# tensor4all/tensor4all-rs

Hardware: AMD Instinct MI355X
Metric: TCI2 full-sweep GF/s (d=30, chi=256 fp64) (higher is better)
Workload: dtype f64

## Files before the change

tensor4all-rs_amd/csrc/engine.hip:

```cpp
#include "engine.hpp"

#include <algorithm>
#include <cmath>
#include <cstdio>
#include <cstdlib>
#include <cstring>
#include <atomic>
#include <condition_variable>
#include <mutex>

namespace t4a {

namespace {
thread_local std::string g_last_error;

__global__ void __launch_bounds__(256) tri_extract_kernel(const double* __restrict__ in, int ldi, int rows, int cols,
                                                          int keep_lower, int unit_diag, double* __restrict__ out,
                                                          int ldo)
{
    const int i = blockIdx.x * blockDim.x + threadIdx.x;
    if (i >= rows) return;
    for (int j = blockIdx.y; j < cols; j += gridDim.y) {
        double v;
        if (i == j)
// ... 249 lines not shown
    if (e != hipSuccess || count <= 0)
        throw Error(T4A_GPU_NO_DEVICE,
                    "no HIP device available: the tensor4all-rs MI355X backend has no CPU fallback (hipGetDeviceCount: " +
                        std::string(hipGetErrorString(e)) + ")");
}

void tri_extract_launch(const double* in, int ldi, int rows, int cols, int keep_lower, int unit_diag, double* out,
                        int ldo, hipStream_t stream)
{
    if (rows <= 0 || cols <= 0) return;
    dim3 grid((rows + 255) / 256, cols < 1024 ? cols : 1024);
    hipLaunchKernelGGL(tri_extract_kernel, grid, dim3(256), 0, stream, in, ldi, rows, cols, keep_lower, unit_diag, out,
                       ldo);
}

Engine::Engine()
{
    require_device();
    num_cus_ = pool::compute_units();
    stream_ = pool::stream_get(1);
    ev_rrlu_.init();
    ev_fac_.init();
    static const int xcc_env = std::getenv("T4A_XCD_ID") ? std::atoi(std::getenv("T4A_XCD_ID")) : -1;
    xcc_ = xcc_env >= 0 ? (xcc_env > 8 ? (xcc_env & 7) : xcc_env) : xcd_assign();
    g_live_engines.fetch_add(1, std::memory_order_relaxed);
    std::call_once(g_census_once, xcd_census);
}

Engine::~Engine()
{
    g_live_engines.fetch_sub(1, std::memory_order_relaxed);
    if (stream_) pool::stream_put(stream_, 1);
}

namespace {
int chain_max_steps(const RrluRoute& rt, size_t max_bond_dim)
{
    const int mn = rt.kM < rt.kN ? rt.kM : rt.kN;
    return max_bond_dim < (size_t)mn ? (int)max_bond_dim : mn;
}
void print_stamps(const RrluRoute& rt, int M, int N, int steps, const unsigned long long* hs)
{
    const double st = steps > 0 ? (double)steps : 1.0;
    switch (rt.kind) {
    case RrluKind::OneWave:
        std::fprintf(stderr, "[rrlu stamps w1] M=%d N=%d columns=%d steps=%d cycles/step: search=%.0f stop+divide+clear=%.0f tables=%.0f update=%.0f | launch (cycles): "
                             "load+init=%llu steps=%llu write-out=%llu | shader clock %.0f MHz\n",
                     M, N, rt.xcd.CPT, steps, hs[0] / st, hs[1] / st, hs[2] / st, hs[3] / st, hs[16], hs[17], hs[18], hs[21] ? 100.0 * (double)hs[20] / (double)hs[21] : 0.0);
        break;
    case RrluKind::OneWorkgroup:
    case RrluKind::SingleXcd:
    case RrluKind::MultiXcd:
        std::fprintf(stderr, "[rrlu stamps xcd] M=%d N=%d W=%d steps=%d cycles/step: pass=%.0f search=%.0f publish=%.0f | prefetch=%.0f keys=%.0f pick=%.0f slow+stop=%.0f recwr=%.0f barB=%.0f | record=%.0f "
                             "tables+u=%.0f colwait=%.0f divide=%.0f barC=%.0f lread=%.0f | pollspins=%llu exact sweeps=%llu exact picks=%llu | launch (cycles): election=%llu load+init=%llu steps=%llu write-out=%llu\n",
                     M, N, rt.xcd.W, steps, hs[0] / st, hs[1] / st, hs[2] / st, hs[6] / st, hs[8] / st, hs[14] / st, hs[15] / st, hs[9] / st, hs[3] / st, hs[10] / st, hs[11] / st, hs[12] / st,
                     hs[4] / st, hs[13] / st, hs[7] / st, hs[5], hs[22], hs[23], hs[16], hs[17], hs[18], hs[19]);
        break;
    default: {
        const bool reg = rt.kind == RrluKind::Reg;
        const int W = reg ? rt.reg.W : rt.kind == RrluKind::Lds ? rt.lds.W : rrlu_global_blocks(M, N);
        const int T = reg ? rt.reg.T : rt.kind == RrluKind::Lds ? rt.lds.T : 256;
        std::fprintf(stderr, "[rrlu stamps %s] M=%d N=%d W=%d T=%d steps=%d | s0=%llu s1=%llu s2=%llu s3=%llu s4=%llu pollspins=%llu colspins=%llu s7=%llu "
                             "(cycles, wg0/thread0; lds: publish,poll,colfetch,pass,reduce; reg: pass,reduce,publish,poll,fetch)\n",
                     reg ? "reg" : "lds", M, N, W, T, steps, hs[0], hs[1], hs[2], hs[3], hs[4], hs[5], hs[6], hs[7]);
    }
    }
}
}

RrluRoute Engine::luci_route(int M, int N, bool left) const
{
    const RrluEnv& env = rrlu_env();
    const bool huge = M > 65535 || N > 65535;
    const int kM = left ? M : N, kN = left ? N : M;
    if (!huge && !env.force_lds && !env.force_global && !env.force_reg && !nonfinite_retry_) {
        RrluXcdPlan xplan;
        if ((long)kM * kN > env.wg_min && (rrlu_w1_make_plan(kM, kN, &xplan, 0) || rrlu_wg_make_plan(kM, kN, &xplan, 0)))
            return RrluRoute::of_xcd(xplan, kM, kN);
        if (!xcd_disabled() && (rrlu_xcd_make_plan(kM, kN, &xplan, false, xcd_plan_max_w()) || rrlu_xcd_make_plan(kM, kN, &xplan, false, 32, true)))
            return RrluRoute::of_xcd(xplan, kM, kN);
    }
    RrluRegPlan rplan;
    if (!huge && !env.force_lds && !env.force_global && rrlu_reg_make_plan(kM, kN, num_cus_, &rplan)) return RrluRoute::of_reg(rplan, kM, kN);
    RrluRoute rt;
    rt.kM = M;
    rt.kN = N;
    if (!huge && !env.force_global) rt.lds = rrlu_make_plan(M, N, num_cus_);
    rt.kind = huge || env.force_global || rt.lds.lds_bytes > 160 * 1024 ? RrluKind::Global : RrluKind::Lds;
    return rt;
}

LuciResult Engine::luci(const double* d_a, int M, int N, const RrLUOptions& opts, bool need_factors, bool want_lu_copy,
                        const FusedPi* fused)
{
    const double* const d_a_in = d_a;
    LuciResult r;
    r.M = M;
    r.N = N;
    r.row_perm.resize(M);
    r.col_perm.resize(N);
    for (int i = 0; i < M; ++i) r.row_perm[i] = i;
    for (int j = 0; j < N; ++j) r.col_perm[j] = j;
    if (M == 0 || N == 0) {
        r.rank = 0;
        r.last_error = 0.0;
        r.pivot_errors = {0.0};
        r.has_factors = need_factors;
        return r;
    }
// ... 300 lines not shown
        const double rr = r.rank;
        prof.v[10] += (M - rr) * rr * rr + 2.0 * rr * rr * N;
        r.has_factors = true;
    }
    return r;
}

void Engine::xcd_take_tickets(const RrluXcdPlan& plan, RrluXcdArgs& a)
{
    if (plan.K > 1) {
        a.ticket = d_xticket_.get() + 8;
        a.ticket_base = xcd_ticket_base_multi_;
        xcd_ticket_base_multi_ += (unsigned)(plan.grid / 8);
    } else {
        a.ticket = d_xticket_.get();
        a.ticket_base = xcd_ticket_base_;
        if (!plan.wg) xcd_ticket_base_ += (unsigned)(plan.grid / 8);
    }
}

void Engine::xcd_mailbox_clear(size_t words, hipStream_t stream)
{
    d_xkeys_.reserve(words);
    d_xticket_.reserve(16);
    T4A_HIP(hipMemsetAsync(d_xkeys_.get(), 0, d_xkeys_.cap * sizeof(unsigned long long), stream));
    T4A_HIP(hipMemsetAsync(d_xticket_.get(), 0, 16 * sizeof(unsigned), stream));
    xcd_ticket_base_ = xcd_ticket_base_multi_ = 0;
    xcd_salt_ = 0;
}

void Engine::xcd_args(RrluXcdArgs& a, const RrluRoute& rt, bool left, const double* A, int max_steps, double rel_tol, double abs_tol,
                      const RrluBlock& blk, int xcc)
{
    std::memset(&a, 0, sizeof(a));
    a.A = A;
    a.M = rt.kM;
    a.N = rt.kN;
    a.max_steps = max_steps;
    a.rel_tol = rel_tol;
    a.abs_tol = abs_tol;
    a.tie_row_major = left ? 0 : 1;
    a.out_transposed = left ? 0 : 1;
    a.W = rt.xcd.W;
    a.xcc = xcc;
    xcd_take_tickets(rt.xcd, a);
    a.row_perm = left ? blk.row_perm() : blk.col_perm();
    a.col_perm = left ? blk.col_perm() : blk.row_perm();
    a.iresult = blk.iresult();
    a.dresult = blk.dresult();
    a.pivot_vals = blk.pivot_vals();
    a.keys = d_xkeys_.get();
    a.salt = xcd_salt_;
    a.spec_frac = 0.8;
    a.h_block = reinterpret_cast<unsigned long long*>(blk.host);
    a.block_u64 = (int)(blk.bytes / 8);
    a.ts_u64 = (int)(blk.off_ts / 8);
}

void Engine::rrlu_account(const RrluRoute& rt, bool tie_row_major, int M, int N, int rank, bool record, float ms, bool saturated)
{
    double bytes = 8.0 * M * N, flops = 0.0;
    for (int k = 0; k < rank; ++k) {
        const double mr = (double)(M - k - 1), nr = (double)(N - k - 1);
        bytes += 16.0 * mr * nr;
        flops += 2.0 * mr * nr + mr;
    }
    prof.v[8] += rank;
    prof.v[9] += bytes;
    prof.v[10] += flops;
    if (!record) return;
    auto add = [&](int code) {
        auto& vs = variant_stats_[code];
        vs[0] += ms;
        vs[1] += 1.0;
        vs[2] += bytes;
        vs[3] += rank;
    };
    add(rt.code(tie_row_major));
    if (saturated) add(rt.code(tie_row_major, true));
}

RrluRoute Engine::chain_route(int kM, int kN) const
{
    if (kM < 1 || kN < 1 || kM > 65535 || kN > 65535) return RrluRoute();
    RrluXcdPlan xplan;
    if ((long long)kM * kN > rrlu_env().wg_min && (rrlu_w1_make_plan(kM, kN, &xplan, 63) || rrlu_wg_make_plan(kM, kN, &xplan, 63)))
        return RrluRoute::of_xcd(xplan, kM, kN);
    RrluRegPlan rplan;
    if ((long long)kM * kN <= 64 * 64 && rrlu_reg_make_plan(kM, kN, num_cus_, &rplan) && rplan.W == 1) return RrluRoute::of_reg(rplan, kM, kN);
    if (!xcd_disabled() && (rrlu_xcd_make_plan(kM, kN, &xplan, true, xcd_plan_max_w()) || rrlu_xcd_make_plan(kM, kN, &xplan, true, 32, true)))
        return RrluRoute::of_xcd(xplan, kM, kN);
    return RrluRoute();
}

void Engine::chain_begin(const std::vector<RrluRoute>& routes, size_t reserve_mailbox_words)
{
    chain_group_reserve(routes, reserve_mailbox_words, stream_);
    RrluLock scope = RrluLock::None;
    for (const RrluRoute& rt : routes)
        if (rt.on_xcd()) scope = std::max(scope, rt.lock());
    acquire_for(chain_lock_, scope, xcc_);
}

void Engine::chain_end() { chain_lock_.release(); }

RrluRoute Engine::chain_group_route(int kM, int kN)
// ... 345 lines not shown
```

tensor4all-rs_amd/csrc/kernels.hpp:

```cpp
#pragma once

#include <hip/hip_runtime.h>

#include <cstddef>
#include <cstdint>

#include "../../include/t4a_testfunctions.h"

namespace t4a {

struct RrluWorkspace;

struct RrluPlan {
    int W = 1;
    int T = 256;
    int cpw = 0;
    int Mld = 0;
    size_t lds_bytes = 0;
};

RrluPlan rrlu_make_plan(int M, int N, int num_cus);

struct RrluArgs {
    const double* A;
// ... 95 lines not shown
    unsigned done_token;
    const int* dims;
    int dims_swap;
    unsigned dev_token;
    const int* rowmap;
    int ts_u64;
};
bool rrlu_reg_make_plan(int M, int N, int num_cus, RrluRegPlan* out);
size_t rrlu_reg_keys_bytes(const RrluRegPlan& plan);
size_t rrlu_reg_cols_bytes(const RrluRegPlan& plan, int M);
void rrlu_reg_launch(const RrluRegPlan& plan, const RrluRegArgs& args, hipStream_t stream, bool keys_zeroed = false);

struct XcdSpecArgs {
    double* out;
    const uint64_t* dep_acc;
    const uint64_t* w_site;
    const uint64_t* ext_acc;
    const int* ext_cnt;
    const uint64_t* ind_acc;
    const int* ind_cnt;
    unsigned* tile_counter;
    int total, d;
    FnDevice fn;
};
struct RrluXcdPlan {
    int W = 1;
    int RPT = 1, CPT = 1;
    int grid = 8;
    size_t lds_bytes = 0;
    int wg = 0;
    int K = 1;
    bool big() const { return K > 1 || RPT > 16; }
};
struct RrluXcdArgs {
    const double* A;
    double* Aout;
    double* urows;
    int M, N;
    int max_steps;
    double rel_tol, abs_tol;
    int tie_row_major;
    int out_transposed;
    int W;
    int xcc;
    unsigned* ticket;
    unsigned ticket_base;
    int* row_perm;
    int* col_perm;
    int* iresult;
    double* dresult;
    double* pivot_vals;
    unsigned long long* keys;
    unsigned salt;
    double spec_frac;
    unsigned long long* stamps;
    unsigned long long* h_block;
    int block_u64;
    const int* dims;
    int dims_swap;
    const int* rowmap;
    XcdSpecArgs spec;
    int ts_u64;
};
bool rrlu_xcd_make_plan(int M, int N, RrluXcdPlan* out, bool any_size = false, int max_w = 32, bool allow_big = false);
size_t rrlu_xcd_keys_bytes(const RrluXcdPlan& plan);
size_t rrlu_xcd_cols_bytes(const RrluXcdPlan& plan, int M);
struct RrluXcdGroupArgs {
    RrluXcdArgs p[8];
};
void rrlu_xcd2_launch(const RrluXcdPlan& plan, const RrluXcdArgs& args, hipStream_t stream);
void rrlu_xcd2m_launch(const RrluXcdPlan& plan, const RrluXcdArgs& args, hipStream_t stream);
void rrlu_xcd2_group_launch(const RrluXcdPlan& plan, const RrluXcdGroupArgs& args, bool tie_row_major, hipStream_t stream);
bool rrlu_wg_make_plan(int M, int N, RrluXcdPlan* out, int spec_blocks = 0);
void rrlu_wg_launch(const RrluXcdPlan& plan, const RrluXcdArgs& args, hipStream_t stream);
void rrlu_wg_group_launch(const RrluXcdPlan& plan, const RrluXcdGroupArgs& args, bool tie_row_major, hipStream_t stream);
bool rrlu_w1_make_plan(int M, int N, RrluXcdPlan* out, int spec_blocks = 0);
void rrlu_w1_launch(const RrluXcdPlan& plan, const RrluXcdArgs& args, hipStream_t stream);
void rrlu_w1_group_launch(const RrluXcdPlan& plan, const RrluXcdGroupArgs& args, bool tie_row_major, hipStream_t stream);

void pi_eval_launch(const FnDevice& fn, const uint64_t* rowacc, int M, const uint64_t* colacc, int N, double* out,
                    int ld, bool transpose_out, unsigned long long* max_abs_bits, hipStream_t stream);
struct PiJob {
    const uint64_t* rowacc;
    const uint64_t* colacc;
    double* out;
    unsigned long long* max_abs_bits;
    int M, N, ld, pad_;
};
void pi_eval_batched_launch(const FnDevice& fn, const PiJob* d_jobs, int n_jobs, int max_M, int max_N, hipStream_t stream);
struct PackJob {
    const double* src;
    double* core;
    const int* info;
    int ld, L, S, R, last, pad_;
};
struct LuProblem;
constexpr int FILL_SMALL_MAX_N = 32, FILL_SMALL_MAX_RHS = 64;
void fill_small_launch(const FnDevice& fn, const PiJob* d_pis, const LuProblem* d_lups, const PackJob* d_packs, int n_jobs, int last_site,
                       hipStream_t stream);
void stage_copy_launch(const uint64_t* pinned_src, uint64_t* dst, size_t count, hipStream_t stream);
void absmax_launch(const double* data, size_t count, unsigned long long* max_abs_bits, hipStream_t stream);

constexpr int CHAIN_MAX_SET = 1024;
struct ChainTab {
    uint64_t* code;
    uint64_t* acc;
// ... 290 lines not shown
```

tensor4all-rs_amd/csrc/kernels_rrlu_xcd2.hip:

```cpp
#include "kernels_rrlu_xcd_common.hpp"

namespace t4a {

namespace {

template <int RPT, int KX = 1> struct Xcd2Lds {
    static constexpr int LSTR = xcd_lstr(RPT);
    static constexpr int TBL = xcd2_tbl(RPT, KX);
    static constexpr int o_l = 0;
    static constexpr int o_wd = o_l + 64 * LSTR * 8;
    static constexpr int o_wi = o_wd + 16;
    static constexpr int o_pp = o_wi + 64;
    static constexpr int o_st = o_pp + 16;
    static constexpr int o_pv = o_st + 128;
    static constexpr int o_pr = o_pv + TBL * 8;
    static constexpr int o_rp = o_pr + TBL * 2;
    static constexpr int o_pc = o_rp + TBL * 2;
    static constexpr int o_cp = o_pc + TBL * 2;
    static constexpr int bytes = o_cp + TBL * 2;
};
static_assert(Xcd2Lds<12>::bytes == (int)xcd_lds_total(12), "plan.lds_bytes must cover the layout");
static_assert(Xcd2Lds<24>::bytes == (int)xcd2_lds_total(24), "plan.lds_bytes must cover the layout (plans beyond 1024 rows)");
static_assert(Xcd2Lds<16, 3>::bytes == (int)xcd2_lds_total(16, 3), "plan.lds_bytes must cover the layout (plans beyond 1024 columns)");

#ifndef T4A_XCD_STAMP_WAVE
#define T4A_XCD_STAMP_WAVE 0
#endif

constexpr unsigned X2_META_VALID = 1u << 13;
constexpr unsigned X2_ROW_MASK = 2047u;
constexpr int X2_QSHIFT = 11, X2_PSHIFT = 11;

constexpr int X2_DIVW = XWAVES - 1;

template <int R0, int NR, int RPT> __device__ __forceinline__ unsigned x2_colmax_hi(unsigned acc, const XSlab<RPT>& col)
{
#pragma unroll
    for (int r = 0; r + 1 < NR; r += 2) acc = vmax3_hi_abs(acc, hi32(col.get(R0 + r)), hi32(col.get(R0 + r + 1)));
    if constexpr ((NR & 1) != 0) acc = vmax3_hi_abs(acc, hi32(col.get(R0 + NR - 1)), hi32(col.get(R0 + NR - 1)));
    return acc;
}

template <int RPT, int CPT, bool ROWMAJOR, int KX = 1>
__device__ __forceinline__ void rrlu_xcd2_body(const RrluXcdArgs& p, const RrluXcdArgs* pk)
{
    static_assert(XWAVES == 8, "the second-generation kernel is written for eight waves per workgroup");
    static_assert(KX >= 1 && KX <= 3, "instantiated for up to three XCDs");
    constexpr int ST_AUX = KX > 1 ? BUF_SC1 : 0;
    extern __shared__ __attribute__((aligned(16))) char smem_raw[];
    using L = Xcd2Lds<RPT, KX>;
    constexpr int LSTR = L::LSTR;
    constexpr int MP = 64 * RPT;
    double* const lbuf = reinterpret_cast<double*>(smem_raw + L::o_l);
    int* const ctl = reinterpret_cast<int*>(smem_raw + L::o_wi);
    unsigned long long* const lds_ptrs = reinterpret_cast<unsigned long long*>(smem_raw + L::o_pp);
    unsigned long long* const lds_stamps = reinterpret_cast<unsigned long long*>(smem_raw + L::o_st);
    double* const lds_pivots = reinterpret_cast<double*>(smem_raw + L::o_pv);
    unsigned short* const posrow = reinterpret_cast<unsigned short*>(smem_raw + L::o_pr);
    unsigned short* const rowpos = reinterpret_cast<unsigned short*>(smem_raw + L::o_rp);
    unsigned short* const poscol = reinterpret_cast<unsigned short*>(smem_raw + L::o_pc);
    unsigned short* const colpos = reinterpret_cast<unsigned short*>(smem_raw + L::o_cp);

    const int tid = threadIdx.x;
    const int lane = tid & 63;
    const int wave = __builtin_amdgcn_readfirstlane(tid >> 6);
    const unsigned long long t_entry = (kXcdStamps && p.stamps) ? __builtin_amdgcn_s_memtime() : 0ull;

    if (tid == 0) {
        int rank = -1;
        if constexpr (KX == 1) {
            if ((int)xcc_id() == p.xcc) {
                const unsigned t = atomicAdd(p.ticket, 1u) - p.ticket_base;
                if (t < (unsigned)p.W) rank = (int)t;
            }
        } else {
            const unsigned x = xcc_id() & 7u;
            const unsigned t = atomicAdd(p.ticket + x, 1u) - p.ticket_base;
            const unsigned xi = (x - (unsigned)p.xcc) & 7u;
            if (xi < (unsigned)KX && t < (unsigned)p.W) rank = (int)(xi * (unsigned)p.W + t);
        }
        ctl[3] = rank;
        ctl[0] = 0;
        ctl[1] = 0;
        ctl[2] = 0;
        for (int e = 8; e < 16; ++e) ctl[e] = 0;
        lds_ptrs[0] = (unsigned long long)p.iresult;
        lds_ptrs[1] = (unsigned long long)p.h_block;
        for (int e = 0; e < 16; ++e) lds_stamps[e] = 0ull;
    }
    __syncthreads();
    const int rank = __builtin_amdgcn_readfirstlane(ctl[3]);
    if (rank < 0) {
        if (p.spec.out && p.dims) {
            const int m_spec = p.dims[2] != 0 ? 0 : (p.dims_swap ? p.dims[1] : p.dims[0]);
            if (m_spec > 0 && m_spec <= p.M)
                xcd_spec_work(reinterpret_cast<const XcdSpecArgs*>(kernarg_base() + offsetof(RrluXcdArgs, spec)), m_spec, ctl + 8);
        }
        return;
    }
    const unsigned long long ts_begin = p.ts_u64 > 0 ? wall_clock64() : 0ull;
    const unsigned long long t_elected = (kXcdStamps && p.stamps) ? __builtin_amdgcn_s_memtime() : 0ull;
    const int NWL = p.W * XWAVES;
    const int NW = KX * NWL;
    const int g = rank * XWAVES + wave;
    const bool poller = wave == 0;
    const int xi = KX > 1 ? rank / p.W : 0;
    const int pbase = xi * NWL;
    int M = p.M, N = p.N, max_steps = p.max_steps;
    int lda = p.M;
    if (p.dims) {
        const int d0 = __builtin_amdgcn_readfirstlane(p.dims[0]), d1 = __builtin_amdgcn_readfirstlane(p.dims[1]);
        M = p.dims_swap ? d1 : d0;
        N = p.dims_swap ? d0 : d1;
        if (M > p.M || N > p.N) M = N = 0;
        const int mn = M < N ? M : N;
        max_steps = max_steps < mn ? max_steps : mn;
        if (mn <= 0) return;
        lda = p.rowmap ? __builtin_amdgcn_readfirstlane(p.dims[3]) : M;
    }
    M = __builtin_amdgcn_readfirstlane(M);
    N = __builtin_amdgcn_readfirstlane(N);
    max_steps = __builtin_amdgcn_readfirstlane(max_steps);
    lda = __builtin_amdgcn_readfirstlane(lda);

    unsigned active = 0u;
#pragma unroll
    for (int q = 0; q < CPT; ++q)
        if (g + NW * q < N) active |= 1u << q;
    XSlab<RPT> a[CPT];
    double local_sqmax = 0.0;
    bool bad = false;
    int srow[RPT];
    unsigned rowmask = 0u;
#pragma unroll
    for (int r = 0; r < RPT; ++r) {
        const int i = lane + 64 * r;
        const bool rok = i < M;
// ... 12 lines not shown
#pragma unroll
    for (int q = 0; q < CPT; ++q) {
        const bool cok = g + NW * q < N;
        const unsigned rm = (unsigned)opaque_v((int)rowmask);
#pragma unroll
        for (int r = 0; r < RPT; ++r) {
            const bool ok = cok && ((rm >> r) & 1u);
            const double v = ok ? a[q].get(r) : 0.0;
            const double sqv = v * v;
            if (sqv > local_sqmax) local_sqmax = sqv;
            bad |= !((v - v) == 0.0);
            a[q].set(r, v);
        }
    }
    bad |= !(local_sqmax < __builtin_huge_val());
    for (int i = tid; i < M; i += XT) {
        posrow[i] = (unsigned short)i;
        rowpos[i] = (unsigned short)i;
    }
    for (int j = tid; j < N; j += XT) {
        poscol[j] = (unsigned short)j;
        colpos[j] = (unsigned short)j;
    }
    for (int e = tid; e < 64 * LSTR; e += XT) lbuf[e] = 0.0;
    {
        const double wm = wave_max_f64(sqrt(local_sqmax));
        if (lane == 0 && wm > 0.0)
            atomicMax((unsigned long long*)&p.dresult[1], (unsigned long long)__double_as_longlong(wm));
    }
    const unsigned wave_bad = __ballot(bad) != 0ull ? 1u : 0u;
    __syncthreads();

    const bool stamp_on = kXcdStamps && (p.stamps != nullptr) && rank == 0 && tid == 64 * T4A_XCD_STAMP_WAVE;
    unsigned long long stamp_last = stamp_on ? __builtin_amdgcn_s_memtime() : 0ull;
    const unsigned long long t_loop = stamp_last;

    const unsigned k2_base = 2u * (unsigned)NW * 16u;
    const unsigned cols_base = 4u * (unsigned)NW * 16u;
    const unsigned fin_base = cols_base + 2u * (unsigned)NW * (unsigned)(MP / 16) * 256u;
    const unsigned k3_base = fin_base + 256u;
    const __amdgpu_buffer_rsrc_t mail =
        __builtin_amdgcn_make_buffer_rsrc((void*)p.keys, 0, (int)(k3_base + (KX > 1 ? 2u * (unsigned)NW * 16u : 0u)), 0x00020000);

    int npiv = 0;
    double max_error = 0.0;
    double error = __builtin_nan("");
    bool timed_out = false;
    const double min_pivot_abs = (p.rel_tol == 0.0 && p.abs_tol == 0.0) ? 0.0 : 2.220446049250313e-16;
    double u[CPT];
#pragma unroll
    for (int q = 0; q < CPT; ++q) u[q] = 0.0;
    double prev_sq = __builtin_huge_val();
    double spec_frac = p.spec_frac, rel_tol_v = p.rel_tol, abs_tol_v = p.abs_tol;
    asm volatile("" : "+v"(spec_frac), "+v"(rel_tol_v), "+v"(abs_tol_v));
    constexpr unsigned XSPIN = 1u << 20;

    unsigned mq[CPT];
#pragma unroll
    for (int q = 0; q < CPT; ++q) mq[q] = (active & (1u << q)) ? x2_colmax_hi<0, RPT>(0u, a[q]) : 0u;
    [[maybe_unused]] unsigned long long n_exact_sweep = 0ull, n_exact_pick = 0ull;
    constexpr int XR = (RPT + X2_DIVW - 1) / X2_DIVW;
    const int sr0 = wave - 1;

    for (int kn = 0; kn < max_steps; ++kn) {
        const int k = kn - 1;
        const int par = kn & 1;
        const unsigned tag = (p.salt << 16) | (unsigned)(kn + 1);
        int mh = (int)mq[0];
#pragma unroll
        for (int q = 1; q < CPT; ++q) mh = (int)mq[q] > mh ? (int)mq[q] : mh;
        const int whi = wave_max_i32(mh);
        const int kslot = (par * NW + g) * 16;
        {
            u32x4 kv;
            kv.x = 0u;
            kv.y = (unsigned)whi;
            kv.z = wave_bad;
            kv.w = tag ^ kv.y ^ kv.z;
            if (lane == 0) __builtin_amdgcn_raw_buffer_store_b128(kv, mail, kslot, 0, 0);
        }
        u32x4 kg[4], kh[4];
        bool has_cand = false;
        double cval = 0.0;
        int cirow = 0, qstar = 0;
        double sq = 0.0;
        if (active != 0u) {
            bool done = false;
            if (hi_mid(whi)) {
                unsigned long long bq[CPT];
                int nhit = 0;
#pragma unroll
                for (int q = 0; q < CPT; ++q) {
                    bq[q] = __ballot(mq[q] == (unsigned)whi);
                    nhit += __builtin_popcountll(bq[q]);
                }
                if (nhit == 1) {
#pragma unroll
                    for (int q = 0; q < CPT; ++q)
                        if (bq[q] != 0ull) {
                            const int hl = (int)__builtin_ctzll(bq[q]);
                            unsigned bits = 0u;
#pragma unroll
                            for (int r = 0; r < RPT; ++r)
                                asm("v_cmp_eq_f32 vcc, |%1|, %2\n\tv_addc_co_u32 %0, vcc, %0, %0, vcc" : "+v"(bits) : "v"(hi32(a[q].get(r))), "s"(whi) : "vcc");
                            const unsigned hb_ = (unsigned)__builtin_amdgcn_readlane((int)bits, hl);
                            if (__builtin_popcount(hb_) == 1) {
                                const int rstar = RPT - 1 - (int)__builtin_ctz(hb_);
// ... 27 lines not shown
                    if (active & (1u << q)) {
                        const unsigned cp_ = colpos[opaque_s(g + NW * q)];
                        auto sweep = [&](int r, double av) {
                            const int i = lane_o + 64 * r;
                            const unsigned rp_ = rowpos[i < M_o ? i : 0];
                            const unsigned key = ROWMAJOR ? ((rp_ << X2_PSHIFT) | cp_) : ((cp_ << X2_PSHIFT) | rp_);
                            const double sc = av * av;
                            const bool hit = (i < M_o) & ((int)rp_ > k) & (sc == sq);
                            if (hit && key < mypos) {
                                mypos = key;
                                myval = av;
                                myrow = i;
                                myq = q;
                            }
                        };
                        if constexpr (RPT <= 16) {
#pragma unroll
                            for (int r = 0; r < RPT; ++r) sweep(r, a[q].get(r));
                        } else {
#pragma unroll 1
                            for (int r = 0; r < RPT; ++r) sweep(r, a[q].dyn(opaque_s(r)));
                        }
                    }
                }
                const unsigned wp = (unsigned)__builtin_amdgcn_readfirstlane((int)wave_min_u32(mypos));
                if (wp != XNOPOS) {
                    const unsigned long long sel = __ballot(mypos == wp);
                    const int hl = (int)__builtin_ctzll(sel);
                    has_cand = true;
                    cval = readlane_f64(myval, hl);
                    cirow = __builtin_amdgcn_readlane(myrow, hl);
                    qstar = __builtin_amdgcn_readlane(myq, hl);
                }
            }
        }
        XSTAMP(1);
        {
            const unsigned meta = (unsigned)cirow | ((unsigned)qstar << X2_QSHIFT) | (has_cand ? X2_META_VALID : 0u);
            u32x4 kv;
            kv.x = lo32(cval);
            kv.y = hi32(cval);
            kv.z = meta;
            kv.w = tag ^ kv.x ^ kv.y ^ meta;
            if (lane == 0) {
                __builtin_amdgcn_raw_buffer_store_b128(kv, mail, (int)k2_base + kslot, 0, 0);
                if constexpr (KX > 1) __builtin_amdgcn_raw_buffer_store_b128(kv, mail, (int)k3_base + kslot, 0, ST_AUX);
            }
        }
        if (poller) {
#pragma unroll
            for (int j = 0; j < 4; ++j)
                kg[j] = __builtin_amdgcn_raw_buffer_load_b128(mail, (par * NW + pbase + min(lane + 64 * j, NWL - 1)) * 16, 0, BUF_SC1);
        }
        const bool early_pub = !poller && has_cand && (sq >= spec_frac * prev_sq);
        constexpr int CS = 256, SLOTB = (MP / 16) * CS;
        const int myslot = (int)cols_base + (par * NW + g) * SLOTB + (lane >> 4) * CS + (lane & 15) * 16;
        if (early_pub) {
            if (qstar == 0) xcd_publish_column<0, RPT, ST_AUX>(a[0], mail, myslot, tag, 4 * CS);
            if constexpr (CPT > 1) if (qstar == 1) xcd_publish_column<1, RPT, ST_AUX>(a[1], mail, myslot, tag, 4 * CS);
            if constexpr (CPT > 2) if (qstar == 2) xcd_publish_column<2, RPT, ST_AUX>(a[2], mail, myslot, tag, 4 * CS);
            if constexpr (CPT > 3) if (qstar == 3) xcd_publish_column<3, RPT, ST_AUX>(a[3], mail, myslot, tag, 4 * CS);
        }
        XSTAMP(2);

        if (poller) {
            unsigned spins = 0;
            int giveup = 0;
            XSTAMP(6);
            for (;;) {
                bool ok = true;
#pragma unroll
                for (int j = 0; j < 4; ++j) ok &= ((kg[j].x ^ kg[j].y ^ kg[j].z ^ kg[j].w) == tag);
                if (__all(ok)) break;
                xcd_poll_again();
                if (++spins > XSPIN) {
                    giveup = 1;
                    break;
                }
#pragma unroll
                for (int j = 0; j < 4; ++j)
                    kg[j] = __builtin_amdgcn_raw_buffer_load_b128(mail, (par * NW + pbase + min(lane + 64 * j, NWL - 1)) * 16, 0, BUF_SC1);
            }
            if (stamp_on) lds_stamps[5] += spins;
            u32x4 fr;
            int xr = 0, fslot = 0;
            if constexpr (KX > 1) {
                fslot = (int)fin_base + (par * KX) * 16;
                xr = (lane < KX && lane != xi) ? lane : (xi == 0 ? 1 : 0);
                fr = __builtin_amdgcn_raw_buffer_load_b128(mail, fslot + xr * 16, 0, BUF_SC1);
            }
#pragma unroll
            for (int j = 0; j < 4; ++j)
                kh[j] = __builtin_amdgcn_raw_buffer_load_b128(mail, (int)k2_base + (par * NW + pbase + min(lane + 64 * j, NWL - 1)) * 16, 0, BUF_SC1);
            XSTAMP(8);
            int wa_ = 0;
            unsigned wkx = 0u, wky = 0u, wkz = 0u;
            if (!giveup) {
                if (kn == 0) {
                    unsigned zf = 0u;
#pragma unroll
                    for (int j = 0; j < 4; ++j) zf |= kg[j].z;
                    if (__ballot(zf != 0u) != 0ull) giveup = 2;
                }
                bool decided = false;
                int lh = (int)kg[0].y;
#pragma unroll
                for (int j = 1; j < 4; ++j) lh = (int)kg[j].y > lh ? (int)kg[j].y : lh;
                const int ghi = wave_max_i32(lh);
                unsigned long long hb[4];
                int nh = 0;
#pragma unroll
                for (int j = 0; j < 4; ++j) {
                    hb[j] = __ballot((int)kg[j].y == ghi);
                    nh += __builtin_popcountll(hb[j]);
                }
                if (hi_mid(ghi) && nh == 1) {
#pragma unroll
                    for (int j = 0; j < 4; ++j)
                        if (hb[j] != 0ull) {
                            const int hl = (int)__builtin_ctzll(hb[j]);
                            wa_ = hl + 64 * j;
                            for (;;) {
                                wkx = (unsigned)__builtin_amdgcn_readlane((int)kh[j].x, hl);
                                wky = (unsigned)__builtin_amdgcn_readlane((int)kh[j].y, hl);
                                wkz = (unsigned)__builtin_amdgcn_readlane((int)kh[j].z, hl);
                                const unsigned kw = (unsigned)__builtin_amdgcn_readlane((int)kh[j].w, hl);
                                if ((wkx ^ wky ^ wkz ^ kw) == tag) break;
                                xcd_poll_again();
                                if (++spins > XSPIN) {
                                    giveup = 1;
                                    break;
                                }
                                kh[j] = __builtin_amdgcn_raw_buffer_load_b128(mail, (int)k2_base + (par * NW + pbase + min(lane + 64 * j, NWL - 1)) * 16, 0, BUF_SC1);
                            }
                        }
                    decided = true;
                } else if (stamp_on) {
                    ++n_exact_pick;
                }
                XSTAMP(14);
                if constexpr (KX > 1) {
                    if (!decided && !giveup) {
                        wkz = 0x80000000u;
                        decided = true;
                    }
                }
                if (!decided && !giveup) {
                    for (;;) {
                        bool ok = true;
#pragma unroll
                        for (int j = 0; j < 4; ++j) ok &= ((kh[j].x ^ kh[j].y ^ kh[j].z ^ kh[j].w) == tag);
                        if (__all(ok)) break;
                        xcd_poll_again();
                        if (++spins > XSPIN) {
                            giveup = 1;
                            break;
                        }
#pragma unroll
                        for (int j = 0; j < 4; ++j)
                            kh[j] = __builtin_amdgcn_raw_buffer_load_b128(mail, (int)k2_base + (par * NW + pbase + min(lane + 64 * j, NWL - 1)) * 16, 0, BUF_SC1);
                    }
// ... 141 lines not shown
                    ctl[1] = giveup;
                    atomicExch(reinterpret_cast<int*>(lds_ptrs[0]) + 1, giveup);
                    if (lds_ptrs[1]) reinterpret_cast<volatile int*>(lds_ptrs[1])[5] = giveup;
                }
                int4 rec;
                rec.x = wa_ | (giveup << 30);
                rec.y = (int)wkx;
                rec.z = (int)wky;
                rec.w = (int)wkz;
                *reinterpret_cast<int4*>(ctl + 4) = rec;
            }
            XSTAMP(9);
        }
        __syncthreads();
        XSTAMP(3);
        int4 rec;
        {
            int zero = 0;
            asm volatile("ds_read_b128 %0, %1 offset:%2\n\ts_waitcnt lgkmcnt(0)" : "=&v"(rec) : "v"(zero), "n"(L::o_wi + 16) : "memory");
        }
        const unsigned recw = (unsigned)__builtin_amdgcn_readfirstlane(rec.x);
        if (recw >> 30) {
            timed_out = true;
            break;
        }
        const int wag = (int)recw;
        if (g == wag && !early_pub) {
            if (qstar == 0) xcd_publish_column<0, RPT, ST_AUX>(a[0], mail, myslot, tag, 4 * CS);
            if constexpr (CPT > 1) if (qstar == 1) xcd_publish_column<1, RPT, ST_AUX>(a[1], mail, myslot, tag, 4 * CS);
            if constexpr (CPT > 2) if (qstar == 2) xcd_publish_column<2, RPT, ST_AUX>(a[2], mail, myslot, tag, 4 * CS);
            if constexpr (CPT > 3) if (qstar == 3) xcd_publish_column<3, RPT, ST_AUX>(a[3], mail, myslot, tag, 4 * CS);
        }
        const int slot_off = (int)cols_base + (par * NW + wag) * SLOTB + ((lane >> 4) + 4 * sr0) * CS + (lane & 15) * 16;
        u32x4 cc[XR];
#pragma unroll
        for (int j = 0; j < XR; ++j)
            if (sr0 >= 0 && sr0 + X2_DIVW * j < RPT) cc[j] = __builtin_amdgcn_raw_buffer_load_b128(mail, slot_off + j * X2_DIVW * 4 * CS, 0, BUF_SC1);
        int rk_ = 0, ck_ = 0;
        int prp_ = 0, pcp_ = 0;
        if (wave == 0) {
            rk_ = posrow[kn];
            ck_ = poscol[kn];
            prp_ = rowpos[rec.w & (int)X2_ROW_MASK];
            pcp_ = colpos[min(wag + NW * ((rec.w >> X2_QSHIFT) & 3), N - 1)];
        }
        const double wval = mk_f64((unsigned)__builtin_amdgcn_readfirstlane(rec.y), (unsigned)__builtin_amdgcn_readfirstlane(rec.z));
        const unsigned wmeta = (unsigned)__builtin_amdgcn_readfirstlane(rec.w);
        const int irow_p = (int)(wmeta & X2_ROW_MASK);
        const int qslot = (int)((wmeta >> X2_QSHIFT) & 3u);
        XSTAMP(10);
        const bool p_mid = exp_mid(wval);
        double rp = refined_rcp(wval);
        asm volatile("" : "+v"(rp));
        prev_sq = wval * wval;
        {
            const int ls = irow_p & 63, rs = irow_p >> 6;
            double ue[CPT];
#pragma unroll
            for (int q = 0; q < CPT; ++q) ue[q] = a[q].dyn(rs);
#pragma unroll
            for (int q = 0; q < CPT; ++q) u[q] = readlane_f64(ue[q], ls);
            if (p.urows) {
#pragma unroll
                for (int q = 0; q < CPT; ++q)
                    if ((active & (1u << q)) && lane == ls) p.urows[(unsigned)(kn * N + (g + NW * q))] = u[q];
            }
        }
        if (g == wag) active &= ~(1u << qslot);
        if (wave == 0) {
            const double wsq = wval * wval;
            double pivot_abs = __builtin_fabs(wval);
            if (!(wsq >= 2.2250738585072014e-308 && wsq < __builtin_huge_val())) pivot_abs = sqrt(mk_f64((unsigned)opaque_v((int)lo32(wsq)), hi32(wsq)));
            error = pivot_abs;
            int stop = 0;
            if (kn > 0 && (pivot_abs < rel_tol_v * max_error || pivot_abs < abs_tol_v)) stop = 1;
            else if (pivot_abs <= min_pivot_abs) stop = 1;
            else max_error = fmax(max_error, pivot_abs);
            if (lane == 0) {
                if (stop) {
                    ctl[0] = 1;
                } else {
                    const int prp = prp_, pcp = pcp_;
                    const int pc = wag + NW * qslot;
                    posrow[prp] = (unsigned short)rk_;
                    posrow[kn] = (unsigned short)irow_p;
                    rowpos[rk_] = (unsigned short)prp;
                    rowpos[irow_p] = (unsigned short)kn;
                    poscol[pcp] = (unsigned short)ck_;
                    poscol[kn] = (unsigned short)pc;
                    colpos[ck_] = (unsigned short)pcp;
                    colpos[pc] = (unsigned short)kn;
                    lds_pivots[kn] = wval;
                }
            }
        }
        XSTAMP(11);

        if (sr0 >= 0) {
            unsigned spins = 0;
            for (;;) {
                bool ok = true;
#pragma unroll
                for (int j = 0; j < XR; ++j)
                    if (sr0 + X2_DIVW * j < RPT) ok &= ((cc[j].x ^ cc[j].y ^ cc[j].z ^ cc[j].w) == tag);
                if (__all(ok)) break;
                xcd_poll_again();
                if (++spins > XSPIN) {
                    atomicExch(reinterpret_cast<int*>(lds_ptrs[0]) + 1, 1);
                    if (lds_ptrs[1]) reinterpret_cast<volatile int*>(lds_ptrs[1])[5] = 1;
                    ctl[1] = 1;
                    break;
                }
#pragma unroll
                for (int j = 0; j < XR; ++j)
                    if (sr0 + X2_DIVW * j < RPT) cc[j] = __builtin_amdgcn_raw_buffer_load_b128(mail, slot_off + j * X2_DIVW * 4 * CS, 0, BUF_SC1);
            }
            XSTAMP(12);
            double lq[XR];
            bool slow = false;
#pragma unroll
            for (int j = 0; j < XR; ++j) {
                lq[j] = 0.0;
                if (sr0 + X2_DIVW * j < RPT) {
                    const double x = mk_f64(cc[j].x, cc[j].y);
                    const double q0 = x * rp;
                    const double qf = __builtin_fma(__builtin_fma(-wval, q0, x), rp, q0);
                    lq[j] = (x == 0.0) ? q0 : qf;
                    slow |= (__builtin_fabs(x) < 4.909093465297727e-91) & (x != 0.0);
                }
            }
            slow |= !p_mid;
            if (__ballot(slow) != 0ull) {
#pragma unroll
                for (int j = 0; j < XR; ++j)
                    if (sr0 + X2_DIVW * j < RPT) {
                        const double x = mk_f64(cc[j].x, cc[j].y);
                        if (!(p_mid & (exp_mid(x) | (x == 0.0)))) lq[j] = x / wval;
                    }
            }
#pragma unroll
            for (int j = 0; j < XR; ++j)
                if (sr0 + X2_DIVW * j < RPT) lbuf[lane * LSTR + sr0 + X2_DIVW * j] = lq[j];
        }
        XSTAMP(4);
        __syncthreads();
        XSTAMP(13);
        int2 fl;
        {
            static_assert(L::o_wi % 8 == 0, "the verdict pair is read with one 8-byte LDS load");
            int zero = 0;
            asm volatile("ds_read_b64 %0, %1 offset:%2" : "=&v"(fl) : "v"(zero), "n"(L::o_wi) : "memory");
        }
        constexpr int NH = RPT > 16 ? 2 : 1, HR = RPT / NH;
        static_assert(RPT % NH == 0, "row slots split evenly into the halves of the l read");
        xvec<HR> l;
#pragma unroll
        for (int r = 0; r < HR; ++r) l[r] = lbuf[lane * LSTR + r];
        {
            asm volatile("s_waitcnt lgkmcnt(%1)" : "+v"(fl) : "n"((HR + 1) / 2) : "memory");
            if (__builtin_amdgcn_readfirstlane(fl.y)) {
                timed_out = true;
                break;
            }
            if (__builtin_amdgcn_readfirstlane(fl.x)) break;
        }
        XSTAMP(7);
        if constexpr (NH == 1) {
#pragma unroll
            for (int q = 0; q < CPT; ++q) {
                mq[q] = 0u;
                if (active & (1u << q)) {
#pragma unroll
                    for (int r = 0; r < RPT; ++r) {
                        double t = a[q].get(r);
                        sub_in_place(t, l[r] * u[q]);
                        a[q].set(r, t);
                    }
                    mq[q] = x2_colmax_hi<0, RPT>(0u, a[q]);
                }
            }
        } else {
#pragma unroll
            for (int q = 0; q < CPT; ++q) mq[q] = 0u;
#pragma unroll
            for (int h = 0; h < NH; ++h) {
                if (h > 0) {
                    asm volatile("" ::: "memory");
#pragma unroll
                    for (int r = 0; r < HR; ++r) l[r] = lbuf[lane * LSTR + h * HR + r];
                }
#pragma unroll
                for (int q = 0; q < CPT; ++q) {
                    if (active & (1u << q)) {
#pragma unroll
                        for (int r = 0; r < HR; ++r) {
                            double t = a[q].get(h * HR + r);
                            sub_in_place(t, l[r] * u[q]);
                            a[q].set(h * HR + r, t);
                        }
                        mq[q] = h == 0 ? x2_colmax_hi<0, HR>(mq[q], a[q]) : x2_colmax_hi<HR, HR>(mq[q], a[q]);
                    }
                }
            }
        }
        npiv = kn + 1;
        XSTAMP(0);
    }

    const RrluXcdArgs* pe_ptr = pk;
    asm volatile("" : "+s"(pe_ptr));
    const RrluXcdArgs& pe = *pe_ptr;
    const int Me = opaque_s(M), Ne = opaque_s(N);
    const unsigned long long t_done = stamp_on ? __builtin_amdgcn_s_memtime() : 0ull;
    __syncthreads();
    if (ctl[1]) timed_out = true;
    if (npiv >= (Me < Ne ? Me : Ne)) error = 0.0;
    if (rank == 0 && tid == 0) {
        pe.iresult[0] = npiv;
        pe.dresult[0] = error;
    }
    if (stamp_on) {
        for (int e = 0; e < 16; ++e) pe.stamps[e] = lds_stamps[e];
        pe.stamps[16] = t_elected - t_entry;
        pe.stamps[17] = t_loop - t_elected;
        pe.stamps[18] = t_done - t_loop;
        pe.stamps[22] = n_exact_sweep;
        pe.stamps[23] = n_exact_pick;
    }
    if (timed_out) return;
    if (rank == 0) {
        int* const h_rp = pe.h_block ? reinterpret_cast<int*>(reinterpret_cast<char*>(pe.h_block) + (reinterpret_cast<const char*>(pe.row_perm) - reinterpret_cast<const char*>(pe.dresult))) : nullptr;
        int* const h_cp = pe.h_block ? reinterpret_cast<int*>(reinterpret_cast<char*>(pe.h_block) + (reinterpret_cast<const char*>(pe.col_perm) - reinterpret_cast<const char*>(pe.dresult))) : nullptr;
        for (int i = tid; i < Me; i += XT) {
            const int v = posrow[i];
            pe.row_perm[i] = v;
            if (h_rp) h_rp[i] = v;
        }
        for (int j = tid; j < Ne; j += XT) {
            const int v = poscol[j];
            pe.col_perm[j] = v;
            if (h_cp) h_cp[j] = v;
        }
        unsigned long long* const h_pv = pe.h_block ? pe.h_block + (reinterpret_cast<const char*>(pe.pivot_vals) - reinterpret_cast<const char*>(pe.dresult)) / 8 : nullptr;
        for (int e = tid; e < npiv; e += XT) {
            const double v = lds_pivots[e];
            pe.pivot_vals[e] = v;
            if (h_pv) h_pv[e] = (unsigned long long)__double_as_longlong(v);
        }
    }
    int nan_seen = 0;
#pragma unroll
    for (int q = 0; q < CPT; ++q)
#pragma unroll
        for (int r = 0; r < RPT; ++r) {
            const int i = lane + 64 * r;
            if (g + NW * q < Ne && i < Me) {
                const int cp = colpos[g + NW * q], rp = rowpos[i];
                const bool from_u = (rp < npiv) && (cp >= rp);
                double v = a[q].get(r);
                const bool in_l = (cp < npiv) && (rp > cp);
                if (in_l) {
                    const double pv = lds_pivots[cp];
                    v = xcd_div(v, pv, refined_rcp(pv), exp_mid(pv));
                    if (v != v) nan_seen = 1;
                }
                if (pe.Aout) {
                    if (from_u)
                        v = __longlong_as_double((long long)__hip_atomic_load(
                            reinterpret_cast<const unsigned long long*>(pe.urows) + ((size_t)rp * Ne + (g + NW * q)), __ATOMIC_RELAXED,
                            __HIP_MEMORY_SCOPE_AGENT));
                    if (pe.out_transposed)
                        pe.Aout[(size_t)rp * Ne + cp] = v;
                    else
                        pe.Aout[(size_t)cp * Me + rp] = v;
                }
            }
        }
    if (nan_seen) {
        atomicExch(&pe.iresult[2], 1);
        if (pe.h_block) ((volatile int*)pe.h_block)[6] = 1;
// ... 165 lines not shown
```

Before: 329.8.

## Replace ratio-based early-publish test with adaptive key threshold targeting a fixed publisher count

In the single-XCD second-generation rrlu kernel, the decision to publish a candidate early no longer compares the squared pivot against a fraction of the previous pivot. It now compares the high key word against a threshold kept in LDS. After each step the threshold is derived from the winning key minus an adaptive margin, tuned so that about spec_m (16) waves publish. The threshold is broadcast through the widened verdict LDS read. The goal is to cut wasted speculative publishes and missed speculation in the pivot search. The change adds per-step ballot and popcount work and a 16-byte LDS read, and also adds stamp counters for diagnostics.

```diff
diff --git a/tensor4all-rs_amd/csrc/engine.hip b/tensor4all-rs_amd/csrc/engine.hip
--- a/tensor4all-rs_amd/csrc/engine.hip
+++ b/tensor4all-rs_amd/csrc/engine.hip
@@ -325,9 +325,9 @@
     case RrluKind::SingleXcd:
     case RrluKind::MultiXcd:
         std::fprintf(stderr, "[rrlu stamps xcd] M=%d N=%d W=%d steps=%d cycles/step: pass=%.0f search=%.0f publish=%.0f | prefetch=%.0f keys=%.0f pick=%.0f slow+stop=%.0f recwr=%.0f barB=%.0f | record=%.0f "
-                             "tables+u=%.0f colwait=%.0f divide=%.0f barC=%.0f lread=%.0f | pollspins=%llu exact sweeps=%llu exact picks=%llu | launch (cycles): election=%llu load+init=%llu steps=%llu write-out=%llu\n",
+                             "tables+u=%.0f colwait=%.0f divide=%.0f barC=%.0f lread=%.0f | pollspins=%llu exact sweeps=%llu exact picks=%llu | early publishers/step=%.1f max=%llu winner had published=%llu | launch (cycles): election=%llu load+init=%llu steps=%llu write-out=%llu\n",
                      M, N, rt.xcd.W, steps, hs[0] / st, hs[1] / st, hs[2] / st, hs[6] / st, hs[8] / st, hs[14] / st, hs[15] / st, hs[9] / st, hs[3] / st, hs[10] / st, hs[11] / st, hs[12] / st,
-                     hs[4] / st, hs[13] / st, hs[7] / st, hs[5], hs[22], hs[23], hs[16], hs[17], hs[18], hs[19]);
+                     hs[4] / st, hs[13] / st, hs[7] / st, hs[5], hs[22], hs[23], (double)(hs[20] & 0xFFFFFFFFFFFFull) / st, hs[20] >> 48, hs[21], hs[16], hs[17], hs[18], hs[19]);
         break;
     default: {
         const bool reg = rt.kind == RrluKind::Reg;
@@ -734,6 +734,7 @@
     a.keys = d_xkeys_.get();
     a.salt = xcd_salt_;
     a.spec_frac = 0.8;
+    a.spec_m = 16;
     a.h_block = reinterpret_cast<unsigned long long*>(blk.host);
     a.block_u64 = (int)(blk.bytes / 8);
     a.ts_u64 = (int)(blk.off_ts / 8);
diff --git a/tensor4all-rs_amd/csrc/kernels.hpp b/tensor4all-rs_amd/csrc/kernels.hpp
--- a/tensor4all-rs_amd/csrc/kernels.hpp
+++ b/tensor4all-rs_amd/csrc/kernels.hpp
@@ -171,6 +171,7 @@
     double* pivot_vals;
     unsigned long long* keys;
     unsigned salt;
+    int spec_m;
     double spec_frac;
     unsigned long long* stamps;
     unsigned long long* h_block;
diff --git a/tensor4all-rs_amd/csrc/kernels_rrlu_xcd2.hip b/tensor4all-rs_amd/csrc/kernels_rrlu_xcd2.hip
--- a/tensor4all-rs_amd/csrc/kernels_rrlu_xcd2.hip
+++ b/tensor4all-rs_amd/csrc/kernels_rrlu_xcd2.hip
@@ -32,6 +32,11 @@
 constexpr int X2_QSHIFT = 11, X2_PSHIFT = 11;
 
 constexpr int X2_DIVW = XWAVES - 1;
+#if defined(T4A_XCD_STAMPS) && defined(T4A_XCD_SPEC_FIXED)
+constexpr bool kXcdSpecFixed = true;
+#else
+constexpr bool kXcdSpecFixed = false;
+#endif
 
 template <int R0, int NR, int RPT> __device__ __forceinline__ unsigned x2_colmax_hi(unsigned acc, const XSlab<RPT>& col)
 {
@@ -47,6 +52,7 @@
     static_assert(XWAVES == 8, "the second-generation kernel is written for eight waves per workgroup");
     static_assert(KX >= 1 && KX <= 3, "instantiated for up to three XCDs");
     constexpr int ST_AUX = KX > 1 ? BUF_SC1 : 0;
+    constexpr bool kCap = KX == 1 && !kXcdSpecFixed;
     extern __shared__ __attribute__((aligned(16))) char smem_raw[];
     using L = Xcd2Lds<RPT, KX>;
     constexpr int LSTR = L::LSTR;
@@ -82,7 +88,7 @@
         ctl[3] = rank;
         ctl[0] = 0;
         ctl[1] = 0;
-        ctl[2] = 0;
+        ctl[2] = 0x7FFFFFFF;
         for (int e = 8; e < 16; ++e) ctl[e] = 0;
         lds_ptrs[0] = (unsigned long long)p.iresult;
         lds_ptrs[1] = (unsigned long long)p.h_block;
@@ -201,7 +207,14 @@
     for (int q = 0; q < CPT; ++q) u[q] = 0.0;
     double prev_sq = __builtin_huge_val();
     double spec_frac = p.spec_frac, rel_tol_v = p.rel_tol, abs_tol_v = p.abs_tol;
-    asm volatile("" : "+v"(spec_frac), "+v"(rel_tol_v), "+v"(abs_tol_v));
+    if constexpr (!kCap) asm volatile("" : "+v"(spec_frac));
+    asm volatile("" : "+v"(rel_tol_v), "+v"(abs_tol_v));
+    int spec_thr = 0x7FFFFFFF;
+    int spec_marg = 1 << 17;
+    int spec_m = p.spec_m;
+    if constexpr (kCap) asm volatile("" : "+v"(spec_m));
+    int ghi_keep = 0;
+    [[maybe_unused]] unsigned long long n_pub = 0ull, n_pub_max = 0ull, n_spec_hit = 0ull;
     constexpr unsigned XSPIN = 1u << 20;
 
     unsigned mq[CPT];
@@ -335,7 +348,9 @@
             for (int j = 0; j < 4; ++j)
                 kg[j] = __builtin_amdgcn_raw_buffer_load_b128(mail, (par * NW + pbase + min(lane + 64 * j, NWL - 1)) * 16, 0, BUF_SC1);
         }
-        const bool early_pub = !poller && has_cand && (sq >= spec_frac * prev_sq);
+        bool early_pub;
+        if constexpr (kCap) early_pub = !poller && has_cand && (whi >= spec_thr);
+        else early_pub = !poller && has_cand && (sq >= spec_frac * prev_sq);
         constexpr int CS = 256, SLOTB = (MP / 16) * CS;
         const int myslot = (int)cols_base + (par * NW + g) * SLOTB + (lane >> 4) * CS + (lane & 15) * 16;
         if (early_pub) {
@@ -390,6 +405,7 @@
 #pragma unroll
                 for (int j = 1; j < 4; ++j) lh = (int)kg[j].y > lh ? (int)kg[j].y : lh;
                 const int ghi = wave_max_i32(lh);
+                ghi_keep = ghi;
                 unsigned long long hb[4];
                 int nh = 0;
 #pragma unroll
@@ -637,7 +653,8 @@
         const bool p_mid = exp_mid(wval);
         double rp = refined_rcp(wval);
         asm volatile("" : "+v"(rp));
-        prev_sq = wval * wval;
+        [[maybe_unused]] const double prev_sq_step = prev_sq;
+        if constexpr (!kCap) prev_sq = wval * wval;
         {
             const int ls = irow_p & 63, rs = irow_p >> 6;
             double ue[CPT];
@@ -678,6 +695,31 @@
                     lds_pivots[kn] = wval;
                 }
             }
+            if constexpr (KX == 1 && kXcdStamps) {
+                if (stamp_on) {
+                    int thr_used = spec_thr;
+                    if constexpr (!kCap) thr_used = prev_sq_step < __builtin_huge_val() ? (int)hi32(sqrt(spec_frac * prev_sq_step)) : 0x7FFFFFFF;
+                    unsigned np = 0u;
+#pragma unroll
+                    for (int j = 0; j < 4; ++j)
+                        np += (unsigned)__builtin_popcountll(__ballot((lane + 64 * j < NWL) && (((lane + 64 * j) & (XWAVES - 1)) != 0) && ((int)kg[j].y >= thr_used)));
+                    n_pub += np;
+                    n_pub_max = np > n_pub_max ? np : n_pub_max;
+                    if ((wag & (XWAVES - 1)) != 0 && ghi_keep >= thr_used) ++n_spec_hit;
+                }
+            }
+            if constexpr (kCap) {
+                const int thr_now = ghi_keep - spec_marg;
+                int cnt = 0;
+#pragma unroll
+                for (int j = 0; j < 4; ++j) cnt += __builtin_popcountll(__ballot((lane + 64 * j < NWL) && ((int)kg[j].y >= thr_now)));
+                const bool miss = kn > 0 && ghi_keep < spec_thr;
+                const int m_ = __builtin_amdgcn_readfirstlane(spec_m);
+                if (miss || cnt < m_) spec_marg += (spec_marg >> 2) + 1;
+                else if (cnt > m_) spec_marg -= spec_marg >> 3;
+                spec_marg = spec_marg > (1 << 20) ? (1 << 20) : spec_marg;
+                if (lane == 0) ctl[2] = ghi_keep - spec_marg;
+            }
         }
         XSTAMP(11);
 
@@ -731,10 +773,12 @@
         __syncthreads();
         XSTAMP(13);
         int2 fl;
+        u32x4 flw;
         {
-            static_assert(L::o_wi % 8 == 0, "the verdict pair is read with one 8-byte LDS load");
+            static_assert(L::o_wi % 16 == 0, "the verdict pair is read with one 8-byte (16-byte) LDS load");
             int zero = 0;
-            asm volatile("ds_read_b64 %0, %1 offset:%2" : "=&v"(fl) : "v"(zero), "n"(L::o_wi) : "memory");
+            if constexpr (kCap) asm volatile("ds_read_b128 %0, %1 offset:%2" : "=&v"(flw) : "v"(zero), "n"(L::o_wi) : "memory");
+            else asm volatile("ds_read_b64 %0, %1 offset:%2" : "=&v"(fl) : "v"(zero), "n"(L::o_wi) : "memory");
         }
         constexpr int NH = RPT > 16 ? 2 : 1, HR = RPT / NH;
         static_assert(RPT % NH == 0, "row slots split evenly into the halves of the l read");
@@ -742,7 +786,14 @@
 #pragma unroll
         for (int r = 0; r < HR; ++r) l[r] = lbuf[lane * LSTR + r];
         {
-            asm volatile("s_waitcnt lgkmcnt(%1)" : "+v"(fl) : "n"((HR + 1) / 2) : "memory");
+            if constexpr (kCap) {
+                asm volatile("s_waitcnt lgkmcnt(%1)" : "+v"(flw) : "n"((HR + 1) / 2) : "memory");
+                fl.x = (int)flw.x;
+                fl.y = (int)flw.y;
+                spec_thr = __builtin_amdgcn_readfirstlane((int)flw.z);
+            } else {
+                asm volatile("s_waitcnt lgkmcnt(%1)" : "+v"(fl) : "n"((HR + 1) / 2) : "memory");
+            }
             if (__builtin_amdgcn_readfirstlane(fl.y)) {
                 timed_out = true;
                 break;
@@ -811,6 +862,8 @@
         pe.stamps[18] = t_done - t_loop;
         pe.stamps[22] = n_exact_sweep;
         pe.stamps[23] = n_exact_pick;
+        pe.stamps[20] = n_pub | (n_pub_max << 48);
+        pe.stamps[21] = n_spec_hit;
     }
     if (timed_out) return;
     if (rank == 0) {
```

Result: slower. 322.9 (-2.1%).
